# medical-genomics-group/ci-gwas

Measured on AMD Instinct MI355X. Metric: ci_tests_per_sec, higher is better.
Workload: dtype f32; 1 GPU; cusk level sweep, one LD block 10000 SNPs x 20 traits, N=16384, alpha=0.0001, max level 5 (north_star headline); correlation matrix from synthetic .bed (Kendall-npn/Pearson) resident in HBM; n_variables=10020, engine=cusk

## Files before the change

### ci-gwas_amd/csrc/cusk_internal.h

```cpp
#pragma once
#include <hip/hip_runtime.h>

#include <cstdint>
#include <cstdio>
#include <string>
#include <vector>

#include "../../include/cusk_hip.h"

namespace cusk {

constexpr int kML = CUSK_ML;
constexpr int kLevels = CUSK_ML + 2;
constexpr unsigned long long kNone = ~0ull;
constexpr int kNumClasses = 5;
constexpr int kClassCap[kNumClasses] = {39, 63, 127, 191, 1 << 30};
constexpr int kThreads = 256;
constexpr int kTmajMinLevelDefault = 6;
constexpr int kCounterSlots = 512;
constexpr size_t kLdsLimit = 160 * 1024;

struct DevBuf
{
    void *p = nullptr;
    size_t cap = 0;
    hipError_t ensure(size_t bytes)
    {
        if (bytes <= cap) return hipSuccess;
        if (p) (void)hipFree(p);
        p = nullptr;
        cap = 0;
        size_t want = bytes + bytes / 4 + 256;
        hipError_t e = hipMalloc(&p, want);
        if (e == hipSuccess) cap = want;
        return e;
    }
    void release()
    {
        if (p) (void)hipFree(p);
        p = nullptr;
        cap = 0;
    }
    template <typename T>
    T *as() const
    {
        return reinterpret_cast<T *>(p);
    }
};

struct LevelCounters;
struct HostGate;

}

struct cusk_engine
{
    int device = 0;
    hipStream_t stream = nullptr;
    hipStream_t stream2 = nullptr;
    hipStream_t stream3 = nullptr;
    float *mxp_pinned = nullptr;
    size_t mxp_pinned_cap = 0, mxp_pending = 0;
    hipEvent_t ev_fork = nullptr, ev_join = nullptr, ev_z = nullptr;
    hipEvent_t ev_mxp = nullptr;
    bool own_stream = false;
    std::string err;

    int n = 0;
    int words = 0;
    int mode = -1;
    bool have_result = false;
    cusk::DevBuf adj, adj0;
    cusk::DevBuf deg, binom, counters, slots, rec_base, ti, queue, symflag;
    cusk::DevBuf off[2], nbr[2], best[2];
    cusk::DevBuf planblk;
    unsigned plan_seq = 0;
    cusk::DevBuf off1;
    cusk::DevBuf items[2][cusk::kNumClasses];
    cusk::DevBuf rec_x, rec_y, rec_l, rec_s;
    long long rec_cap = 0;
    long long rec_slots = 0;
    cusk::DevBuf den_x, den_y, den_l, den_z, den_s, den_counts, den_off;
    long long den_stride = 0;
    bool records_ready = false, z_ready = false;
    cusk::DevBuf scratch_a, scratch_b;
    const float *last_C = nullptr;
    int last_levels = 0;
    std::vector<int> batch_lo, batch_hi;
    cusk::DevBuf row_range, row_blk, blk_woff;
    void *batch_pinned = nullptr;
    size_t batch_pinned_cap = 0;
    void *res_pinned = nullptr;
    size_t res_pinned_cap = 0;
    cusk::DevBuf rv, rpos, sel, wpre;
    cusk::DevBuf nv;
    int level1_form = -1;
    long long nrec = 0;
    cusk::LevelCounters *hcnt = nullptr;
    unsigned long long *hslots = nullptr;
    long long *hrec_base = nullptr;
    unsigned long long *hcanon = nullptr;
    int *hflag = nullptr;
    std::vector<unsigned long long> binom_host;
    long long binom_rows = 0;
    cusk::HostGate *hgate = nullptr, *hgate_dev = nullptr;
    int run_seq = 0;
    long long item_cap_cur = 0;
    hipEvent_t ev_main[2] = {nullptr, nullptr};
    hipEvent_t ev_run[2] = {nullptr, nullptr};
    hipEvent_t ev_k0[cusk::kLevels], ev_k1[cusk::kLevels], ev_l0[cusk::kLevels], ev_l1[cusk::kLevels];

    int opt_fast = 1;
    int opt_validate = 0;
    int opt_het_filter = 0;
    int opt_het_rows = 0;
    int opt_corr_fp4 = 1;
    int opt_pair = 1;
    int opt_rows = 1;
    int opt_vec = 1;
    int opt_overlap = 1;
    int opt_corr_popcount = 0;
    int opt_corr_mxp_f32 = 0;
    int opt_assume_symmetric = 0;
    long long opt_queue_cap = 4ll << 20;
    int opt_hostprof = 0;
    int opt_tmaj_validate_stride = 1;
    int opt_max_staged_classes = -1;
    int opt_tmaj_min_level = cusk::kTmajMinLevelDefault;
    long long opt_chunk = 2048;
    long long opt_chunk0 = 512;
    long long opt_chunk0_low = 256;
    int opt_vec_threads = 64;
    long long opt_item_cap = 1ll << 20;
    int opt_lookahead = 2;
    int opt_sync2 = 1;
    int opt_l1_threads = 0;
    int opt_l1_lds_row = 1;
    int opt_timing = 1;
    long long opt_sep_ws_budget = 4ll << 30;

    int shard_rank = 0, shard_world = 1;
    int shard_host_staging = 0;
    cusk_exchange_fn shard_fn = nullptr;
    void *shard_user = nullptr;
    void *shard_host = nullptr;
    size_t shard_host_cap = 0;

    cusk::DevBuf bed_dev, phen_dev, mean_dev, std_dev, planes, mxp_dev, pxp_dev, mxp_bq;
    cusk::DevBuf pc_masks, pc_counts;
    cusk::DevBuf mp_bits;
    cusk::DevBuf corr_tab[2];
    void *corr_tab_pinned[2] = {nullptr, nullptr};
    size_t corr_tab_pinned_cap[2] = {0, 0};
    hipEvent_t ev_corr[5] = {nullptr, nullptr, nullptr, nullptr, nullptr};
    float corr_ms[4] = {0, 0, 0, 0};
};

namespace cusk {

inline int fail(cusk_engine *e, int code, const std::string &msg)
{
    if (e) e->err = msg;
    return code;
}

#define CUSK_HIP(e, call)                                                                        \
    do                                                                                           \
    {                                                                                            \
        hipError_t _st = (call);                                                                 \
        if (_st != hipSuccess)                                                                   \
            return cusk::fail((e), CUSK_ERR_HIP,                                                 \
                              std::string(#call) + ": " + hipGetErrorString(_st) + " (" +        \
                                  __FILE__ + ":" + std::to_string(__LINE__) + ")");              \
    } while (0)

void threshold_array_host(int n, float alpha, float *thr15);
float hetcor_threshold_host(float alpha);

int corr_build_impl(cusk_engine *e, const unsigned char *bed, const float *phen, size_t m, size_t N,
                    size_t p, const float *mean, const float *std, float *C_dev, float *mxp_host,
                    float *mxm_tri_host, float *pxp_tri_host, bool ahead = false);
bool is_device_pointer(const void *p);

int check_marker_ix(cusk_engine *e, const int *marker_ix, size_t k, size_t m_total);
int pack_bed_rows(cusk_engine *e, const unsigned char *bed, const int *marker_ix, const int *&ix_d, size_t k, size_t m_total,
                  size_t clb, std::vector<unsigned char> &bed_h, const unsigned char *&bed_k);

void compat_marker_phen_corr_pearson(const unsigned char *marker_vals, const float *phen_vals, const size_t num_markers,
                                     const size_t num_individuals, const size_t num_phen, const float *marker_mean,
                                     const float *marker_std, float *marker_phen_corrs);
void compat_corr_pearson_npn(const unsigned char *marker_vals, const float *phen_vals, const size_t num_markers,
                             const size_t num_individuals, const size_t num_phen, const float *marker_mean,
                             const float *marker_std, float *marker_corrs, float *marker_phen_corrs, float *phen_corrs);
double qnorm_host(double p);

}
```

### ci-gwas_amd/csrc/engine.hip

```cpp
#include <algorithm>
#include <atomic>
#include <chrono>
#include <cmath>
#include <cstdlib>
#include <cstring>

#include "sweep_common.h"

namespace cusk {

static unsigned long long binom_sat(int n, int k)
{
    if (k < 0 || k > n) return 0;
    if (k > n - k) k = n - k;
    unsigned long long r = 1;
    const unsigned long long cap = 1ull << 62;
    for (int i = 1; i <= k; i++)
    {
        unsigned long long f = (unsigned long long)(n - k + i);
        if (r > cap / f) return cap;
        r = r * f / (unsigned long long)i;
    }
    return r;
}
// ... 253 lines not shown
        CUSK_HIP(e, launch_finalize(l, pl.fp, s));
        return CUSK_OK;
    };

    auto shard_join = [&](int l) -> int {
        LevelPlan &pl = plan[l];
        if (pl.use_fast && l >= 2)
        {
            CUSK_HIP(e, hipMemcpyAsync(e->hcnt + l, dcnt + l, sizeof(LevelCounters), hipMemcpyDeviceToHost, s));
            CUSK_HIP(e, hipStreamSynchronize(s));
            if (e->hcnt[l].qcount > (unsigned long long)e->opt_queue_cap)
            {
                pl.redone = true;
                local.exact_fallbacks++;
                qcap_gate[l] = ~0ull;
                const int rc = launch_level_sweeps(l, true);
                if (rc != CUSK_OK) return rc;
            }
        }
        const size_t count = (size_t)e->hgate[l].total_edges;
        if (a.mode == 1 && !pl.use_rows) CUSK_HIP(e, launch_marks_from_bitmap(pl.sp, e->sel.as<unsigned>(), s));
        const int elem = (pl.use_rows || a.mode == 1) ? 4 : 8;
        void *dev = (pl.use_rows || a.mode == 1) ? e->sel.p : e->best[l & 1].p;
        int rc = 0;
        if (e->shard_host_staging)
        {
            const size_t bytes = count * (size_t)elem;
            if (bytes > e->shard_host_cap)
            {
                if (e->shard_host) (void)hipHostFree(e->shard_host);
                e->shard_host = nullptr;
                e->shard_host_cap = 0;
                CUSK_HIP(e, hipHostMalloc(&e->shard_host, std::max<size_t>(bytes, 64)));
                e->shard_host_cap = std::max<size_t>(bytes, 64);
            }
            CUSK_HIP(e, hipMemcpyAsync(e->shard_host, dev, bytes, hipMemcpyDeviceToHost, s));
            CUSK_HIP(e, hipStreamSynchronize(s));
            rc = e->shard_fn(e->shard_user, l, e->shard_host, count, elem, 0, (void *)s);
            if (rc == 0) CUSK_HIP(e, hipMemcpyAsync(dev, e->shard_host, bytes, hipMemcpyHostToDevice, s));
        }
        else
        {
            CUSK_HIP(e, hipStreamSynchronize(s));
            rc = e->shard_fn(e->shard_user, l, dev, count, elem, 1, (void *)s);
        }
        if (rc != 0) return fail(e, CUSK_ERR_ARG, "row-shard exchange failed at level " + std::to_string(l));
        if (a.mode == 1)
            CUSK_HIP(e, launch_level1_apply(pl.sp, e->sel.as<unsigned>(), (l == 1 && pl.use_rows) ? e->rpos.p : nullptr, false, s));
        return CUSK_OK;
    };

    if (last_level >= 1 && !a.row_range)
        CUSK_HIP(e, launch_degree(e->adj.as<unsigned long long>(), e->deg.as<int>(), n, words,
                                  a.mode == 0 ? e->adj0.as<unsigned long long>() : nullptr, s));

    int staged_classes = 0;
    while (staged_classes < kNumClasses - 1 && lds_layout(kClassCap[staged_classes], het).total <= kLdsLimit) staged_classes++;
    if (e->opt_max_staged_classes >= 0) staged_classes = std::min(staged_classes, e->opt_max_staged_classes);
    const int lookahead = sharded ? 0 : std::max(0, e->opt_lookahead);
    auto wait_gate = [&](int l) -> int {
        volatile int *seq = &e->hgate[l].seq;
        for (unsigned long it = 1; *seq != run_seq; it++)
        {
            if ((it & 0x3fff) == 0)
            {
                const hipError_t q = hipStreamQuery(s);
                if (q == hipSuccess)
                {
                    if (*seq == run_seq) break;
                    return fail(e, CUSK_ERR_HIP, "level " + std::to_string(l) + ": the stream drained without the level's gate record");
                }
                if (q != hipErrorNotReady) return fail(e, CUSK_ERR_HIP, std::string("stream error while waiting for a level gate: ") + hipGetErrorString(q));
            }
            __builtin_ia32_pause();
        }
        std::atomic_thread_fence(std::memory_order_acquire);
        return CUSK_OK;
    };
    int maxdeg1 = 0;
    int maxdeg2 = -1;
    int start = 1;
    int redo = 0;
    bool first_pass = true;

    for (;;)
    {
        if (redo > 0)
        {
            plan[redo].redone = true;
            local.exact_fallbacks++;
            qcap_gate[redo] = ~0ull;
            int rc = launch_level_sweeps(redo, true);
            if (rc != CUSK_OK) return rc;
            rc = launch_level_finalize(redo);
            if (rc != CUSK_OK) return rc;
            if (e->opt_timing == 2) CUSK_HIP(e, hipEventRecord(e->ev_l1[redo], s));
            redo = 0;
        }
        int enq_last = start - 1;
        int planned_last = start - 1;
        for (int l = start; l <= last_level; l++)
        {
            const int cs = l & 1;
            {
                const int k = l - 1 - lookahead;
                if (k >= start)
                {
                    const int rc = wait_gate(k);
                    if (rc != CUSK_OK) return rc;
                    if (!e->hgate[k].active) break;
                }
            }
            if (e->opt_timing == 2) CUSK_HIP(e, hipEventRecord(e->ev_l0[l], s));
            LevelPlan &pl = plan[l];
            pl.redone = false;
            pl.known_items = false;
            const bool first_build = (l == 1 && first_pass);
            int *off_l = (l == 1) ? e->off1.as<int>() : e->off[cs].as<int>();
            PlanArgs pa;
            pa.deg = e->deg.as<int>();
            pa.off = off_l;
            for (int c = 0; c < kNumClasses; c++) pa.items[c] = e->items[cs][c].as<int2>();
            pa.n = n;
            pa.L = l;
            pa.binom = e->binom.as<unsigned long long>();
            pa.chunk = chunk;
            {
                float th_l;
                if (het)
                    th_l = a.Th[0];
                else if (a.mode == 0)
                    th_l = a.Th[l];
                else
                    th_l = uniform_ess_threshold(a.Th[0], a.ess_uniform, l);
                const bool vec0 = (e->opt_fast != 0) && l >= 2 && l < kVecMaxLevel && th_l >= kThMinFilter && !het && e->opt_vec &&
                                  !e->opt_validate && staged_classes > 0;
                const unsigned long long c0 = (l <= 4) ? (unsigned long long)std::max<long long>(e->opt_chunk0_low, 64) : chunk0;
                plan[l].chunk0 = vec0 ? c0 : chunk;
                plan[l].tmaj = (e->opt_fast != 0) && !plan[l].force_exact && l >= std::max(2, e->opt_tmaj_min_level) && l <= kML &&
                               th_l >= kThMinFilter && (!het || ness_symmetric) && symmetric && !sharded;
                if (plan[l].tmaj) plan[l].chunk0 = chunk;
            }
            pa.chunk0 = plan[l].chunk0;
            pa.Lsets = plan[l].tmaj ? l + 1 : l;
            pa.staged_classes = staged_classes;
            pa.pair_mode = ((l == 1) && !first_build && plan[l].use_pair && !plan[l].use_rows) ? 1 : 0;
            pa.cnt = dcnt + l;
            pa.prev = (l >= 2) ? dcnt + (l - 1) : nullptr;
            pa.prev_qcap = (l >= 2) ? qcap_gate[l - 1] : ~0ull;
            pa.item_cap = item_cap;
            pa.shard_rank = e->shard_rank;
            pa.shard_world = e->shard_world;
            pa.gate = e->hgate_dev + l;
            pa.seq = run_seq;
            pa.sym = (l == 1 && !e->opt_assume_symmetric && !a.row_range) ? dsym : nullptr;
            pa.blocks = e->planblk.as<unsigned long long>();
            pa.blk_seq = ++e->plan_seq;
            if (first_build && e->binom_rows <= 0)
            {
                CUSK_HIP(e, e->binom.ensure(sizeof(unsigned long long) * kBinomStride));
                pa.binom = e->binom.as<unsigned long long>();
            }
            CUSK_HIP(e, launch_plan(pa, s));
            planned_last = l;
            if (first_build)
            {
                hp_mark("plan1_enq");
                int *const rec_l_before = (a.mode == 0) ? e->rec_l.as<int>() : nullptr;
                const size_t rec_l_cleared = rec_l_before ? e->rec_l.cap : 0;
                if (rec_l_cleared) CUSK_HIP(e, hipMemsetAsync(rec_l_before, 0, rec_l_cleared, s));
                int rc = wait_gate(1);
                if (rc != CUSK_OK) return rc;
                hp_mark("gate1");
                symmetric = (e->hgate[1].sym == 0) || (e->opt_assume_symmetric != 0) || (a.row_range != nullptr);
                ness_symmetric = ness_checked && (*reinterpret_cast<volatile int *>(e->hflag) == 0);
                ness_symmetric_rows = ness_checked_rows && (*reinterpret_cast<volatile int *>(e->hflag) == 0);
                cap_edges = std::max<long long>(e->hgate[1].total_edges, 1);
                maxdeg1 = e->hgate[1].maxdeg;
                for (int k = 0; k < 2; k++)
                {
                    CUSK_HIP(e, e->nbr[k].ensure(sizeof(int) * ((size_t)cap_edges + 4)));
                    if (a.mode == 0) CUSK_HIP(e, e->best[k].ensure(sizeof(unsigned long long) * (size_t)cap_edges));
                }
                CUSK_HIP(e, e->rv.ensure(sizeof(float) * ((size_t)cap_edges + 4)));
                CUSK_HIP(e, e->rpos.ensure(sizeof(int) * 4 * (size_t)cap_edges));
                CUSK_HIP(e, e->sel.ensure(sizeof(unsigned) * (size_t)cap_edges));
                if (a.mode == 0)
                {
                    CUSK_HIP(e, e->rec_x.ensure(sizeof(int) * (size_t)cap_edges));
                    CUSK_HIP(e, e->rec_y.ensure(sizeof(int) * (size_t)cap_edges));
                    CUSK_HIP(e, e->rec_l.ensure(sizeof(int) * (size_t)cap_edges));
                    CUSK_HIP(e, e->rec_s.ensure(sizeof(int) * kML * (size_t)cap_edges));
                    e->rec_cap = (long long)(e->rec_l.cap / sizeof(int));
                    if ((long long)(e->rec_s.cap / (sizeof(int) * kML)) < e->rec_cap) e->rec_cap = (long long)(e->rec_s.cap / (sizeof(int) * kML));
                    e->rec_slots = cap_edges;
                    if (e->rec_l.as<int>() != rec_l_before || rec_l_cleared < sizeof(int) * (size_t)cap_edges)
                        CUSK_HIP(e, hipMemsetAsync(e->rec_l.p, 0, sizeof(int) * (size_t)cap_edges, s));
                    CUSK_HIP(e, e->wpre.ensure(sizeof(int) * (size_t)n * words));
                }
                CUSK_HIP(e, e->queue.ensure(sizeof(RecheckEntry) * (size_t)e->opt_queue_cap));
                if ((long long)maxdeg1 >= e->binom_rows)
                {
                    const int rows = std::max(maxdeg1 + 1, 1024);
                    e->binom_host.assign((size_t)rows * kBinomStride, 0ull);
                    for (int aa = 0; aa < rows; aa++)
                        for (int b = 0; b < kBinomStride; b++)
                            e->binom_host[(size_t)aa * kBinomStride + b] = binom_sat(aa, b);
                    CUSK_HIP(e, e->binom.ensure(e->binom_host.size() * sizeof(unsigned long long)));
                    CUSK_HIP(e, hipMemcpyAsync(e->binom.p, e->binom_host.data(),
                                               e->binom_host.size() * sizeof(unsigned long long), hipMemcpyHostToDevice, s));
                    e->binom_rows = rows;
                }
                pl.pair_lds = (size_t)maxdeg1 * 20 + 16;
                pl.use_pair = !het && symmetric && (e->opt_pair != 0) && pl.pair_lds <= 64 * 1024;
                pl.use_rows = !het && symmetric && (e->opt_pair != 0) && (e->opt_rows != 0);
                if (het0 && ness_symmetric_rows && symmetric && (e->opt_fast != 0) && (e->opt_pair != 0) && (e->opt_rows != 0))
                {
                    pl.use_rows = true;
                    CUSK_HIP(e, e->nv.ensure(sizeof(float) * ((size_t)cap_edges + 4)));
                }
                if (pl.use_rows) CUSK_HIP(e, e->wpre.ensure(sizeof(int) * (size_t)n * words));
                if (pl.use_pair && !pl.use_rows)
                {
                    CUSK_HIP(e, hipMemsetAsync(dcnt + l, 0, sizeof(LevelCounters), s));
                    pa.pair_mode = 1;
                    pa.binom = e->binom.as<unsigned long long>();
                    pa.seq = run_seq;
                    e->hgate[1].seq = 0;
                    pa.blk_seq = ++e->plan_seq;
                    CUSK_HIP(e, launch_plan(pa, s));
                }
                first_pass = false;
            }
            if (sharded)
            {
                const int rc = wait_gate(l);
                if (rc != CUSK_OK) return rc;
                if (!e->hgate[l].active) break;
                for (int c = 0; c < kNumClasses; c++) pl.nitems[c] = e->hgate[l].class_items[c];
                pl.known_items = true;
            }
            pl.use_fast = (e->opt_fast != 0) && (l >= 2) && !pl.force_exact && !het0_exact;
            CUSK_HIP(e, launch_fill_nbr(e->adj.as<unsigned long long>(), off_l, e->nbr[cs].as<int>(),
                                        (a.mode == 0 && !pl.use_rows) ? e->best[cs].as<unsigned long long>() : nullptr, n, words,
                                        (l == 1 && (pl.use_rows || a.mode == 0)) ? e->wpre.as<int>() : nullptr, dcnt + l, a.row_range, s));
            if (l == 2 && !sharded && e->opt_sync2)
            {
                const int rc2 = wait_gate(2);
                if (rc2 != CUSK_OK) return rc2;
                if (!e->hgate[2].active) break;
                for (int c = 0; c < kNumClasses; c++) pl.nitems[c] = e->hgate[2].class_items[c];
                pl.known_items = !e->hgate[2].item_overflow;
                maxdeg2 = e->hgate[2].maxdeg;
            }
            {
                pl.maxdeg_bound = maxdeg1;
                if (maxdeg2 >= 0 && l >= 2) pl.maxdeg_bound = std::min(pl.maxdeg_bound, maxdeg2);
                const int k = l - 1 - lookahead;
                if (k >= 1 && e->hgate[k].seq == run_seq && e->hgate[k].active) pl.maxdeg_bound = std::min(pl.maxdeg_bound, e->hgate[k].maxdeg);
                pl.staged_classes = staged_classes;
            }

            SweepParams &sp = pl.sp;
            sp.C = a.C;
            sp.Ness = a.Ness;
            sp.n = n;
            sp.level = l;
            sp.off = off_l;
            sp.nbr = e->nbr[cs].as<int>();
            sp.best = e->best[cs].as<unsigned long long>();
            sp.adj = e->adj.as<unsigned long long>();
            sp.deg = e->deg.as<int>();
            sp.words = words;
            sp.items = nullptr;
            sp.binom = e->binom.as<unsigned long long>();
            sp.time_index = e->ti.as<int>();
            sp.has_ti = (a.mode == 1 && a.time_index != nullptr) ? 1 : 0;
            sp.chunk = chunk;
            sp.cap = 0;
            sp.cls = 0;
            sp.item_cap = item_cap;
            sp.grid_cap = item_cap;
            sp.cnt = dcnt + l;
            sp.row_range = a.row_range;
            sp.max_span = a.row_range ? a.max_span : n;
            sp.slots = dslots + (size_t)l * kCounterSlots * 4;
            if (het)
                sp.th = a.Th[0];
            else if (a.mode == 0)
                sp.th = a.Th[l];
            else
                sp.th = uniform_ess_threshold(a.Th[0], a.ess_uniform, l);
            {
                const double tq = std::tanh((double)sp.th);
                sp.t2 = (float)(tq * tq);
                pl.filter_ok = (sp.th >= kThMinFilter);
                if (!pl.filter_ok) pl.use_fast = false;
            }
            sp.queue = nullptr;
            sp.qcap = 0;
            qcap_gate[l] = ~0ull;
            if (pl.use_fast)
            {
                sp.queue = e->queue.as<RecheckEntry>();
                sp.qcap = (unsigned long long)e->opt_queue_cap;
                qcap_gate[l] = sp.qcap;
            }
            FinalizeParams &fp = pl.fp;
            fp.C = a.C;
            fp.n = n;
            fp.off = sp.off;
            fp.nbr = sp.nbr;
            fp.best = sp.best;
            fp.sel = pl.use_rows ? e->sel.as<unsigned>() : nullptr;
            fp.level = l;
            fp.adj = sp.adj;
            fp.deg = sp.deg;
            fp.words = words;
            fp.binom = sp.binom;
            fp.off1 = e->off1.as<int>();
            fp.wpre1 = e->wpre.as<int>();
            fp.adj0 = e->adj0.as<unsigned long long>();
            fp.rec_x = e->rec_x.as<int>();
            fp.rec_y = e->rec_y.as<int>();
            fp.rec_l = e->rec_l.as<int>();
            fp.rec_s = e->rec_s.as<int>();
            fp.rec_cap = e->rec_cap;
            fp.meta = pl.use_rows ? e->rpos.as<int4>() : nullptr;
            fp.cnt = dcnt + l;
            fp.qcap = qcap_gate[l];
            fp.slots = sp.slots;
            fp.canon = dcanon + (size_t)l * kCounterSlots;

            if (e->opt_timing == 1 || e->opt_timing == 2) CUSK_HIP(e, hipEventRecord(e->ev_k0[l], s));
            int rc = launch_level_sweeps(l, false);
            if (rc != CUSK_OK) return rc;
            if (e->opt_timing == 1 || e->opt_timing == 2) CUSK_HIP(e, hipEventRecord(e->ev_k1[l], s));
            if (sharded)
            {
                rc = shard_join(l);
                if (rc != CUSK_OK) return rc;
            }
            rc = launch_level_finalize(l);
            if (rc != CUSK_OK) return rc;
            if (e->opt_timing == 2) CUSK_HIP(e, hipEventRecord(e->ev_l1[l], s));
            enq_last = l;
        }

        CUSK_HIP(e, hipEventRecord(e->ev_join, e->stream2));
        CUSK_HIP(e, hipStreamWaitEvent(s, e->ev_join, 0));
        CUSK_HIP(e, hipMemcpyAsync(e->hcnt, ctl, ctl_sym, hipMemcpyDeviceToHost, s));
        CUSK_HIP(e, hipEventRecord(e->ev_run[1], s));
        hp_mark("all_enq");
        CUSK_HIP(e, hipStreamSynchronize(s));
        hp_mark("synced");
        int ended = 0;
        for (int l = 1; l <= planned_last && !ended; l++)
            if (!e->hcnt[l].active) ended = l;
        const int last_ran = ended ? ended - 1 : enq_last;
        if (!sharded && last_ran >= 2 && plan[last_ran].use_fast && !plan[last_ran].redone &&
            e->hcnt[last_ran].qcount > (unsigned long long)e->opt_queue_cap)
        {
            if (plan[last_ran].tmaj)
            {
                plan[last_ran].force_exact = true;
                local.exact_fallbacks++;
                start = last_ran;
            }
            else
            {
                redo = last_ran;
                start = last_ran + 1;
            }
        }
        else if (ended && e->hcnt[ended].overflow)
            return fail(e, CUSK_ERR_OVERFLOW,
                        "C(degree, level) exceeds 2^62 at level " + std::to_string(ended) + " (max degree " +
                            std::to_string(e->hcnt[ended].maxdeg) + ")");
        else if (ended && e->hcnt[ended].item_overflow)
        {
            long long need = item_cap;
            for (int c = 0; c < kNumClasses; c++) need = std::max(need, e->hcnt[ended].class_items[c]);
            item_cap = need + need / 4;
            for (int k = 0; k < 2; k++)
                for (int c = 0; c < kNumClasses; c++) CUSK_HIP(e, e->items[k][c].ensure(sizeof(int2) * (size_t)item_cap));
            start = ended;
        }
        else
        {
            levels_swept = last_ran;
            if (ended) level_out = ended - 1;
            break;
        }
        for (int l = start; l < kLevels; l++) e->hgate[l].seq = 0;
        if (start <= 2) maxdeg2 = -1;
        if (start <= last_level)
        {
            CUSK_HIP(e, hipMemsetAsync(dcnt + start, 0, sizeof(LevelCounters) * (size_t)(kLevels - start), s));
            CUSK_HIP(e, hipMemsetAsync(dslots + (size_t)start * kCounterSlots * 4, 0,
                                       sizeof(unsigned long long) * (size_t)(kLevels - start) * kCounterSlots * 4, s));
            CUSK_HIP(e, hipMemsetAsync(dcanon + (size_t)start * kCounterSlots, 0,
                                       sizeof(unsigned long long) * (size_t)(kLevels - start) * kCounterSlots, s));
        }
    }
    for (int l = 1; l <= std::min(levels_swept + 1, last_level); l++)
    {
        local.max_degree[l] = e->hcnt[l].maxdeg;
        local.edges[l] = e->hcnt[l].total_edges;
    }
    local.levels_run += levels_swept;
    float ms = 0.0f;
    CUSK_HIP(e, hipEventElapsedTime(&ms, e->ev_l0[0], e->ev_l1[0]));
    local.kernel_ms[0] = local.level_ms[0] = ms;
    const bool timed = (e->opt_timing == 1 || e->opt_timing == 2);
    for (int l = 1; l <= levels_swept; l++)
    {
        for (int k = 0; k < kCounterSlots; k++)
        {
            const unsigned long long *sl = e->hslots + ((size_t)l * kCounterSlots + k) * 4;
            local.tests[l] += (long long)sl[0];
            local.subsets[l] += (long long)sl[1];
            local.removed[l] += (long long)sl[2];
            local.violations += (long long)sl[3];
            if (a.mode == 0 || l == 1) local.canonical_tests[l] += (long long)e->hcanon[(size_t)l * kCounterSlots + k];
        }
        local.rechecks[l] = (long long)e->hcnt[l].qcount;
        if (!timed)
        {
            if (e->opt_timing == 3 && l == 1 && rows_timed)
            {
                CUSK_HIP(e, hipEventElapsedTime(&ms, e->ev_main[0], e->ev_main[1]));
                local.main_kernel_ms[l] = ms;
            }
            continue;
        }
        CUSK_HIP(e, hipEventElapsedTime(&ms, e->ev_k0[l], e->ev_k1[l]));
        local.kernel_ms[l] = ms;
        local.main_kernel_ms[l] = ms;
        if (l == 1 && rows_timed)
        {
            CUSK_HIP(e, hipEventElapsedTime(&ms, e->ev_main[0], e->ev_main[1]));
            local.main_kernel_ms[l] = ms;
        }
// ... 127 lines not shown
    if (e->shard_host) (void)hipHostFree(e->shard_host);
    if (e->hcnt) (void)hipHostFree(e->hcnt);
    if (e->hflag) (void)hipHostFree(e->hflag);
    if (e->hgate) (void)hipHostFree(e->hgate);
    for (auto &ev : e->ev_run)
        if (ev) (void)hipEventDestroy(ev);
    for (auto &ev : e->ev_main)
        if (ev) (void)hipEventDestroy(ev);
    for (auto &ev : e->ev_corr)
        if (ev) (void)hipEventDestroy(ev);
    for (int l = 0; l < kLevels; l++)
        for (hipEvent_t ev : {e->ev_k0[l], e->ev_k1[l], e->ev_l0[l], e->ev_l1[l]})
            if (ev) (void)hipEventDestroy(ev);
    for (hipEvent_t ev : {e->ev_fork, e->ev_join, e->ev_z, e->ev_mxp})
        if (ev) (void)hipEventDestroy(ev);
    if (e->stream2) (void)hipStreamDestroy(e->stream2);
    if (e->stream3) (void)hipStreamDestroy(e->stream3);
    if (e->mxp_pinned) (void)hipHostFree(e->mxp_pinned);
    if (e->own_stream && e->stream) (void)hipStreamDestroy(e->stream);
    delete e;
}

extern "C" int cusk_engine_set_option(cusk_engine *e, const char *key, long long value)
{
    if (!e || !key) return CUSK_ERR_ARG;
    const std::string k(key);
    if (k == "fast")
        e->opt_fast = (int)value;
    else if (k == "validate")
        e->opt_validate = (int)value;
    else if (k == "het_filter")
        e->opt_het_filter = (int)value;
    else if (k == "het_rows" && (value == 0 || value == 1))
        e->opt_het_rows = (int)value;
    else if (k == "corr_fp4")
        e->opt_corr_fp4 = (int)value;
    else if (k == "pair")
        e->opt_pair = (int)value;
    else if (k == "rows")
        e->opt_rows = (int)value;
    else if (k == "vec")
        e->opt_vec = (int)value;
    else if (k == "overlap")
        e->opt_overlap = (int)value;
    else if (k == "corr_popcount")
        e->opt_corr_popcount = (int)value;
    else if (k == "corr_mxp_f32")
        e->opt_corr_mxp_f32 = (int)value;
    else if (k == "assume_symmetric")
        e->opt_assume_symmetric = (int)value;
    else if (k == "queue_capacity" && value > 0)
        e->opt_queue_cap = value;
    else if (k == "chunk" && value >= 256)
        e->opt_chunk = value;
    else if (k == "max_staged_classes")
        e->opt_max_staged_classes = (int)value;
    else if (k == "tmaj_validate_stride" && value >= 1 && (value & (value - 1)) == 0)
        e->opt_tmaj_validate_stride = (int)value;
    else if (k == "tmaj_min_level")
        e->opt_tmaj_min_level = (int)value;
    else if (k == "hostprof")
        e->opt_hostprof = (int)value;
    else if (k == "chunk0_low" && value >= 64)
        e->opt_chunk0_low = value;
    else if (k == "chunk0" && value >= 64)
        e->opt_chunk0 = value;
    else if (k == "vec_threads" && (value == 64 || value == 128 || value == 256))
        e->opt_vec_threads = (int)value;
    else if (k == "item_capacity" && value > 0)
    {
        e->opt_item_cap = value;
        e->item_cap_cur = 0;
    }
    else if (k == "lookahead" && value >= 0)
        e->opt_lookahead = (int)value;
    else if (k == "timing")
        e->opt_timing = (int)value;
    else if (k == "l1_threads" && (value == 0 || value == 256 || value == 512))
        e->opt_l1_threads = (int)value;
    else if (k == "l1_lds_row" && (value == 0 || value == 1))
        e->opt_l1_lds_row = (int)value;
    else if (k == "sync2")
        e->opt_sync2 = (int)value;
    else if (k == "sepselect_ws_bytes" && value > 0)
        e->opt_sep_ws_budget = value;
    else
        return fail(e, CUSK_ERR_ARG, "unknown option " + k);
    return CUSK_OK;
}

extern "C" int cusk_engine_set_row_shard(cusk_engine *e, int rank, int world, cusk_exchange_fn fn, void *user, int host_staging)
{
    if (!e) return CUSK_ERR_ARG;
    if (world < 1 || rank < 0 || rank >= world || (world > 1 && !fn))
        return fail(e, CUSK_ERR_ARG, "cusk_engine_set_row_shard: need 0 <= rank < world and an exchange function");
    e->shard_rank = rank;
    e->shard_world = world;
    e->shard_fn = fn;
    e->shard_user = user;
    e->shard_host_staging = host_staging ? 1 : 0;
    return CUSK_OK;
}

extern "C" const char *cusk_last_error(const cusk_engine *e) { return e ? e->err.c_str() : "no engine"; }
extern "C" void *cusk_engine_stream(const cusk_engine *e) { return e ? (void *)e->stream : nullptr; }
extern "C" int cusk_engine_device(const cusk_engine *e) { return e ? e->device : -1; }
extern "C" int cusk_engine_level1_form(const cusk_engine *e) { return e ? e->level1_form : -1; }
extern "C" int cusk_engine_bind_thread(cusk_engine *e)
{
    if (!e) return CUSK_ERR_ARG;
    CUSK_HIP(e, hipSetDevice(e->device));
    return CUSK_OK;
}

extern "C" int cusk_run_skeleton(cusk_engine *e, const float *C_dev, int n, const float *Th, int maxlevel,
                                 cusk_stats *stats)
{
    if (!e) return CUSK_ERR_ARG;
    e->batch_lo.clear();
    RunArgs a{};
    a.mode = 0;
    a.C = C_dev;
    a.Th = Th;
    a.n = n;
    a.maxlevel = maxlevel;
    return run_levels(e, a, stats);
}

static int batch_setup(cusk_engine *e, const char *who, int n, int nblk, const int *lo, const int *hi, RunArgs &a)
{
    int prev = 0, span = 0;
    long long pairs0 = 0;
    for (int b = 0; b < nblk; b++)
    {
        if ((lo[b] & 63) != 0 || lo[b] < prev || hi[b] < lo[b] || hi[b] > n)
            return fail(e, CUSK_ERR_ARG, std::string(who) + ": block bases must be ascending multiples of 64 inside the matrix");
        prev = hi[b];
        span = std::max(span, hi[b] - lo[b]);
        pairs0 += (long long)(hi[b] - lo[b]) * (hi[b] - lo[b] - 1) / 2;
    }
    CUSK_HIP(e, hipSetDevice(e->device));
    const size_t bytes_rr = sizeof(int2) * (size_t)n, bytes_rb = sizeof(int) * (size_t)n, bytes_wo = sizeof(long long) * (size_t)nblk;
    const size_t need = bytes_rr + bytes_rb + bytes_wo;
    if (need > e->batch_pinned_cap)
    {
        if (e->batch_pinned) (void)hipHostFree(e->batch_pinned);
        e->batch_pinned = nullptr;
        e->batch_pinned_cap = 0;
        CUSK_HIP(e, hipHostMalloc(&e->batch_pinned, need + need / 2));
        e->batch_pinned_cap = need + need / 2;
    }
    int2 *rr = static_cast<int2 *>(e->batch_pinned);
    int *rb = reinterpret_cast<int *>(static_cast<char *>(e->batch_pinned) + bytes_rr);
    long long *wo = reinterpret_cast<long long *>(static_cast<char *>(e->batch_pinned) + bytes_rr + bytes_rb);
    for (int r = 0; r < n; r++)
    {
        rr[r] = make_int2(0, 0);
        rb[r] = -1;
    }
    long long woff = 0;
    for (int b = 0; b < nblk; b++)
    {
        for (int r = lo[b]; r < hi[b]; r++)
        {
            rr[r] = make_int2(lo[b], hi[b]);
            rb[r] = b;
        }
        wo[b] = woff;
        woff += (long long)(hi[b] - lo[b]) * ((hi[b] - lo[b] + 63) / 64);
    }
    CUSK_HIP(e, e->row_range.ensure(bytes_rr));
    CUSK_HIP(e, e->row_blk.ensure(bytes_rb));
    CUSK_HIP(e, e->blk_woff.ensure(bytes_wo));
    CUSK_HIP(e, hipMemcpyAsync(e->row_range.p, rr, bytes_rr, hipMemcpyHostToDevice, e->stream));
    CUSK_HIP(e, hipMemcpyAsync(e->row_blk.p, rb, bytes_rb, hipMemcpyHostToDevice, e->stream));
    CUSK_HIP(e, hipMemcpyAsync(e->blk_woff.p, wo, bytes_wo, hipMemcpyHostToDevice, e->stream));
    e->batch_lo.assign(lo, lo + nblk);
    e->batch_hi.assign(hi, hi + nblk);
    a.row_range = e->row_range.as<int2>();
    a.max_span = span;
    a.level0_pairs = pairs0;
    return CUSK_OK;
}

extern "C" int cusk_run_skeleton_batch(cusk_engine *e, const float *C_dev, int n, int nblk, const int *lo, const int *hi,
                                       const float *Th, int maxlevel, cusk_stats *stats)
{
    if (!e) return CUSK_ERR_ARG;
    if (!C_dev || !lo || !hi || !Th || n <= 0 || nblk <= 0) return fail(e, CUSK_ERR_ARG, "bad arguments");
    if (e->shard_world > 1) return fail(e, CUSK_ERR_ARG, "batched runs are not row-sharded");
// ... 418 lines not shown
```

### ci-gwas_amd/csrc/plan.hip

```cpp
#include "sweep_common.h"

namespace cusk {


__global__ void degree_kernel(const unsigned long long *__restrict__ adj, int *deg, int n, int words, unsigned long long *adj0)
{
    const int row = blockIdx.x * (blockDim.x >> 6) + (threadIdx.x >> 6);
    const int lane = threadIdx.x & 63;
    if (row >= n) return;
    int d = 0;
    for (int w = lane; w < words; w += 64)
    {
        const unsigned long long v = adj[(size_t)row * words + w];
        if (adj0) adj0[(size_t)row * words + w] = v;
        d += __popcll(v);
    }
    for (int o = 32; o > 0; o >>= 1) d += __shfl_xor(d, o);
    if (lane == 0) deg[row] = d;
}

hipError_t launch_degree(const unsigned long long *adj, int *deg, int n, int words, unsigned long long *adj0, hipStream_t st)
{
    hipLaunchKernelGGL(degree_kernel, dim3((n + 3) / 4), dim3(256), 0, st, adj, deg, n, words, adj0);
    return hipGetLastError();
// ... 23 lines not shown
        int incl = c;
        for (int o = 1; o < 64; o <<= 1)
        {
            const int v = __shfl_up(incl, o);
            if (lane >= o) incl += v;
        }
        int pos = o0 + run + incl - c;
        if (wpre && w < w_end) wpre[(size_t)row * words + w] = run + incl - c;
        while (bits)
        {
            const int b = __ffsll((long long)bits) - 1;
            bits &= bits - 1;
            if (best) best[pos] = kNone;
            nbr[pos++] = w * 64 + b;
        }
        run += __shfl(incl, 63);
    }
}

hipError_t launch_fill_nbr(const unsigned long long *adj, const int *off, int *nbr, unsigned long long *best, int n, int words,
                           int *wpre, const LevelCounters *cnt, const int2 *row_range, hipStream_t st)
{
    hipLaunchKernelGGL(fill_nbr_kernel, dim3((n + 3) / 4), dim3(256), 0, st, adj, off, nbr, best, n, words, wpre, cnt, row_range);
    return hipGetLastError();
}

__device__ __forceinline__ long long prefix_256(const int *__restrict__ in, int n, int v, long long *s_red, long long *block_total)
{
    const int tid = threadIdx.x, lane = tid & 63, wave = tid >> 6;
    const int first = blockIdx.x * 256;
    long long before = 0;
    for (int i0 = 0; i0 < first; i0 += 256 * 16)
    {
        int t[16];
#pragma unroll
        for (int u = 0; u < 16; u++)
        {
            const int i = i0 + u * 256 + tid;
            t[u] = (i < first) ? in[i] : 0;
        }
#pragma unroll
        for (int u = 0; u < 16; u++) before += t[u];
    }
    int incl = v;
    for (int o = 1; o < 64; o <<= 1)
    {
        const int t = __shfl_up(incl, o);
        if (lane >= o) incl += t;
    }
    for (int o = 32; o > 0; o >>= 1) before += __shfl_xor(before, o);
    if (lane == 63) s_red[wave] = incl;
    if (lane == 0) s_red[4 + wave] = before;
    __syncthreads();
    long long pre = s_red[4] + s_red[5] + s_red[6] + s_red[7];
    for (int w = 0; w < wave; w++) pre += s_red[w];
    *block_total = s_red[0] + s_red[1] + s_red[2] + s_red[3];
    (void)n;
    return pre + incl - v;
}

constexpr int kPlanWords = 8;
static_assert(kNumClasses + 1 < 7, "plan words");
constexpr unsigned long long kPlanMask = (1ull << 40) - 1ull;

__global__ void __launch_bounds__(256) plan_kernel(PlanArgs a)
{
    __shared__ long long s_wave[kNumClasses][4];
    __shared__ int s_wdeg[4], s_wmax[4];
    __shared__ long long s_part[4][kPlanWords];
    __shared__ long long s_base[kNumClasses];
    __shared__ int s_cls[256], s_nch[256], s_pos[256];
    __shared__ unsigned long long s_big[4];
    LevelCounters *cnt = a.cnt;
    const int n = a.n, L = a.L;
    if (a.prev != nullptr && !level_complete(a.prev, a.prev_qcap))
    {
        if (blockIdx.x == 0 && threadIdx.x == 0)
        {
            HostGate *g = a.gate;
            g->active = 0;
            g->maxdeg = 0;
            g->overflow = 0;
            g->item_overflow = 0;
            g->sym = 0;
            g->total_edges = 0;
            for (int c = 0; c < kNumClasses; c++) g->class_items[c] = 0;
            __threadfence_system();
            *(volatile int *)&g->seq = a.seq;
        }
        return;
    }
    const int tid = threadIdx.x;
    const int row = blockIdx.x * 256 + tid;
    const int lane = tid & 63, wave = tid >> 6;
    int cls = -1, nchunks = 0;
    const int d = (row < n) ? a.deg[row] : 0;
    bool ovf = false;
    if (d > L)
    {
        const unsigned long long nc = a.pair_mode ? (unsigned long long)d * (d - 1) / 2
                                                  : (L == 1 ? (unsigned long long)d : a.binom[(size_t)d * kBinomStride + a.Lsets]);
        if (nc >= (1ull << 62))
            ovf = true;
        else
        {
            cls = 0;
            while (d > kClassCap[cls]) cls++;
            if (cls >= a.staged_classes) cls = kNumClasses - 1;
            const unsigned long long ch = (cls == 0) ? a.chunk0 : a.chunk;
            if (a.Lsets == L + 1 && L >= 2)
            {
                const int np = L - 2;
                long long tot = 0;
                for (int s = np; s <= d - 3; s++)
                {
                    const unsigned long long nP = (np == 0) ? 1ull : a.binom[(size_t)s * kBinomStride + np];
                    const unsigned long long per = (unsigned long long)kThreads * tmaj_prefixes_per_lane(d, s, ch);
                    tot += (long long)((nP + per - 1ull) / per);
                }
                if (tot > (long long)0x7fffffff)
                    ovf = true;
                else
                    nchunks = (int)tot;
            }
            else
            {
                const unsigned long long units = (nc + ch - 1) / ch;
                if (units > 0x7fffffffull)
                    ovf = true;
                else
                    nchunks = (int)units;
            }
            if (ovf || !(a.shard_world == 1 || row % a.shard_world == a.shard_rank))
            {
                cls = -1;
                nchunks = 0;
            }
        }
    }
    const bool wave_ovf = __ballot(ovf) != 0ull;
    int dincl = d, dmax = d;
    for (int o = 1; o < 64; o <<= 1)
    {
        const int t = __shfl_up(dincl, o);
        if (lane >= o) dincl += t;
    }
    for (int o = 32; o > 0; o >>= 1) dmax = max(dmax, __shfl_xor(dmax, o));
    if (lane == 63) s_wdeg[wave] = dincl;
    if (lane == 0) s_wmax[wave] = dmax | (wave_ovf ? (1 << 30) : 0);
    long long excl[kNumClasses];
#pragma unroll
    for (int c = 0; c < kNumClasses; c++)
    {
        const long long mine = (cls == c) ? nchunks : 0;
        long long v = mine;
        for (int o = 1; o < 64; o <<= 1)
        {
            const long long t = __shfl_up(v, o);
            if (lane >= o) v += t;
        }
        excl[c] = v - mine;
        if (lane == 63) s_wave[c][wave] = v;
    }
    __syncthreads();
    unsigned long long *blk = a.blocks + (size_t)blockIdx.x * kPlanWords;
    const unsigned long long tag = (unsigned long long)a.blk_seq << 40;
// ... 24 lines not shown
        }
        for (int o = 8; o < 64; o <<= 1)
        {
            const long long t = __shfl_xor(acc, o);
            acc = (w >= 6) ? max(acc, t) : acc + t;
        }
        if (lane < kPlanWords) s_part[wave][lane] = acc;
    }
    __syncthreads();
    long long before[kPlanWords];
#pragma unroll
    for (int w = 0; w < kPlanWords; w++)
    {
        const long long p0 = s_part[0][w], p1 = s_part[1][w], p2 = s_part[2][w], p3 = s_part[3][w];
        before[w] = (w >= 6) ? max(max(p0, p1), max(p2, p3)) : p0 + p1 + p2 + p3;
    }
    {
        long long o0 = before[0] + dincl - d;
        for (int w = 0; w < wave; w++) o0 += s_wdeg[w];
        if (row < n) a.off[row] = (int)o0;
    }
    const bool last = (blockIdx.x == gridDim.x - 1);
    long long tot_items[kNumClasses];
#pragma unroll
    for (int c = 0; c < kNumClasses; c++)
    {
        const long long mine = s_wave[c][0] + s_wave[c][1] + s_wave[c][2] + s_wave[c][3];
        tot_items[c] = before[1 + c] + mine;
        if (tid == c) s_base[c] = (tot_items[c] > a.item_cap) ? -1 : before[1 + c];
    }
    __syncthreads();
    {
        int pos = -1;
        if (cls >= 0 && s_base[cls] >= 0)
        {
            long long add = 0;
            for (int w = 0; w < wave; w++) add += s_wave[cls][w];
            long long e = 0;
#pragma unroll
            for (int c = 0; c < kNumClasses; c++)
                if (cls == c) e = excl[c];
            pos = (int)(s_base[cls] + add + e);
        }
        const bool big = (pos >= 0 && nchunks > 1);
        if (pos >= 0 && nchunks == 1) a.items[cls][pos] = make_int2(row, 0);
        const unsigned long long bm = __ballot(big);
        if (lane == 0) s_big[wave] = bm;
        if (big)
        {
            s_cls[tid] = cls;
            s_nch[tid] = nchunks;
            s_pos[tid] = pos;
        }
        __syncthreads();
        const int row0 = blockIdx.x * 256;
        for (int w = 0; w < 4; w++)
        {
            unsigned long long m = s_big[w];
            while (m)
            {
                const int r = w * 64 + __builtin_ctzll(m);
                m &= m - 1;
                const int nch = s_nch[r];
                int2 *dst = a.items[s_cls[r]] + s_pos[r];
                for (int c = tid; c < nch; c += 256) dst[c] = make_int2(row0 + r, c);
            }
        }
    }
    if (last && tid == 0)
    {
        const long long edges = before[0] + s_wdeg[0] + s_wdeg[1] + s_wdeg[2] + s_wdeg[3];
        const int maxdeg = (int)max(before[6], (long long)(max(max(s_wmax[0], s_wmax[1]), max(s_wmax[2], s_wmax[3])) & ~(1 << 30)));
        a.off[n] = (int)edges;
        const int ovf_all = (before[7] != 0 || (((s_wmax[0] | s_wmax[1] | s_wmax[2] | s_wmax[3]) >> 30) & 1)) ? 1 : 0;
        cnt->overflow = ovf_all;
        bool fits = true;
        HostGate *g = a.gate;
        for (int c = 0; c < kNumClasses; c++)
        {
            fits = fits && (tot_items[c] <= a.item_cap);
            cnt->class_items[c] = tot_items[c];
            g->class_items[c] = tot_items[c];
        }
        const int active = (maxdeg - 1 >= L && ovf_all == 0 && fits) ? 1 : 0;
        cnt->maxdeg = maxdeg;
        cnt->total_edges = edges;
        cnt->item_overflow = fits ? 0 : 1;
        cnt->active = active;
        g->active = active;
        g->maxdeg = maxdeg;
        g->overflow = ovf_all;
        g->item_overflow = fits ? 0 : 1;
        g->sym = a.sym ? *a.sym : 0;
        g->total_edges = edges;
        __threadfence_system();
        *(volatile int *)&g->seq = a.seq;
    }
}

hipError_t launch_plan(const PlanArgs &a, hipStream_t st)
{
    hipLaunchKernelGGL(plan_kernel, dim3((a.n + 255) / 256), dim3(256), 0, st, a);
    return hipGetLastError();
}

}
```

### ci-gwas_amd/csrc/sweep_common.h

```cpp
#pragma once
#include "cusk_internal.h"

namespace cusk {

constexpr int kBinomStride = 16;
constexpr int kVecMaxLevel = 9;
constexpr float kThMinFilter = 2e-3f;

struct RowInfo
{
    int cls;
    int base;
    int nchunks;
    int pad;
};

struct RecheckEntry
{
    int x;
    int k2;
    unsigned long long rank;
};

struct LevelCounters
{
    int maxdeg;
    int overflow;
    long long total_edges;
    long long class_items[kNumClasses];
    unsigned long long qcount;
    unsigned long long rec_total;
    int active;
    int item_overflow;
    unsigned int done_blocks;
    int pad;
    unsigned long long next_item[kNumClasses];
};

struct HostGate
{
    int seq;
    int active, maxdeg, overflow, item_overflow, sym;
    long long total_edges;
    long long class_items[kNumClasses];
};

struct SweepParams
{
    const float *C;
    const float *Ness;
    int n;
    int level;
    const int *off;
    const int *nbr;
    unsigned long long *best;
    unsigned long long *adj;
    int *deg;
    int words;
    const int2 *items;
    const unsigned long long *binom;
    const int *time_index;
    int has_ti;
    float th;
    float t2;
    unsigned long long chunk;
    int cap;
    int cls;
    long long item_cap;
    long long grid_cap;
    LevelCounters *cnt;
    unsigned long long *slots;
    RecheckEntry *queue;
    unsigned long long qcap;
    int validate;
    const int2 *row_range;
    int max_span;
};

struct FinalizeParams
{
    const float *C;
    int n;
    const int *off;
    const int *nbr;
    const unsigned long long *best;
    const unsigned *sel;
    int level;
    unsigned long long *adj;
    int *deg;
    int words;
    const unsigned long long *binom;
    const int *off1;
    const int *wpre1;
    const unsigned long long *adj0;
    int *rec_x, *rec_y, *rec_l, *rec_s;
    long long rec_cap;
    const int4 *meta;
    const LevelCounters *cnt;
    unsigned long long qcap;
    unsigned long long *slots;
    unsigned long long *canon;
};

__host__ __device__ inline size_t align16(size_t x) { return (x + 15) & ~(size_t)15; }

struct LdsLayout
{
    size_t nbr, best, ti, sub, ess, total;
};
__host__ __device__ inline LdsLayout lds_layout(int cap, bool het)
{
    LdsLayout l;
    size_t ld = (size_t)((cap + 1) | 1);
    l.nbr = 0;
    l.best = align16(l.nbr + sizeof(int) * (cap + 1));
    l.ti = align16(l.best + sizeof(unsigned long long) * cap);
    l.sub = align16(l.ti + sizeof(int) * (cap + 1));
    l.ess = align16(l.sub + sizeof(float) * (cap + 1) * ld);
    l.total = het ? align16(l.ess + sizeof(float) * (cap + 1) * ld) : l.ess;
    return l;
}

#if defined(__HIPCC__)
__device__ __forceinline__ long long level_items(const SweepParams &p)
{
// ... 46 lines not shown
#pragma unroll
    for (int i = 0; i < L; i++)
    {
        const int lo = prev + 1, hi = S[i] - 1;
        const int t = L - i - 1;
        if (lo <= hi)
        {
            if (in_prefix)
                cnt += C(d - lo, t + 1) - C(d - 1 - hi, t + 1);
            else if (k > prev)
            {
                const int h2 = min(hi, k - 1);
                if (t >= 1 && lo <= h2) cnt += C(d - 1 - lo, t) - C(d - 2 - h2, t);
                if (lo <= k && k <= hi) cnt += C(d - 1 - k, t);
            }
        }
        if (S[i] == k) in_prefix = true;
        prev = S[i];
    }
    return cnt + (in_prefix ? 1ull : 0ull);
}

__device__ __forceinline__ bool clear_edge(unsigned long long *adj, int *deg, int words, int X, int Y)
{
    const unsigned long long o1 = atomicAnd(&adj[(size_t)X * words + (Y >> 6)], ~(1ull << (Y & 63)));
    const unsigned long long o2 = atomicAnd(&adj[(size_t)Y * words + (X >> 6)], ~(1ull << (X & 63)));
    const bool f1 = (o1 >> (Y & 63)) & 1ull, f2 = (o2 >> (X & 63)) & 1ull;
    if (f1) atomicSub(&deg[X], 1);
    if (f2) atomicSub(&deg[Y], 1);
    return f1;
}
#endif

hipError_t launch_sweep_exact(int mode, bool het, int L, const SweepParams &p, int cls, hipStream_t st);
hipError_t launch_recheck(int mode, bool het, int L, const SweepParams &p, hipStream_t st);
hipError_t launch_finalize(int L, const FinalizeParams &p, hipStream_t st);
hipError_t launch_record_z(int L, const float *C, int n, const int *x, const int *y, const int *l, const int *s, long long stride,
                           long long count, float *z, hipStream_t st);
constexpr int kRecBlock = 1024;
hipError_t launch_rec_count(const int *rec_l, long long slots, int *counts, hipStream_t st);
hipError_t launch_rec_compact(const int *rec_l, const int *rec_x, const int *rec_y, const int *rec_s, long long rec_cap,
                              long long slots, const long long *block_off, int *out_x, int *out_y, int *out_l, int *out_s,
                              long long out_stride, hipStream_t st);
hipError_t launch_sweep_fast(int mode, bool het, int L, bool validate, const SweepParams &p, int cls, hipStream_t st);
hipError_t launch_sweep_tmaj(int mode, bool het, int L, const SweepParams &p, int cls, hipStream_t st);
hipError_t launch_ess_symmetry(const float *N, int n, const int2 *row_range, int *flag, hipStream_t st);
__host__ __device__ inline int tmaj_prefixes_per_lane(int d, int s, unsigned long long chunk)
{
    const unsigned long long r = (unsigned long long)(d - 1 - s);
    const unsigned long long pairs = r * (r - 1ull) / 2ull;
    const unsigned long long k = chunk / ((unsigned long long)kThreads * (pairs ? pairs : 1ull));
    return (int)(k < 1ull ? 1ull : (k > 64ull ? 64ull : k));
}
hipError_t launch_sweep_vec(int mode, int L, const SweepParams &p, int cls, int threads, hipStream_t st);
unsigned persistent_grid(const void *kernel, int threads, size_t lds);
size_t sweep_vec_lds_bytes(int cls);
hipError_t launch_level0(const float *C, const float *Ness, const int *Ginit, unsigned long long *adj, int n, int words,
                         float th, int *asym_flag, hipStream_t st);
hipError_t launch_level0_batch(const float *C, const float *Ness, unsigned long long *adj, unsigned long long *adj0, int *deg, int n,
                               int words, const int2 *row_range, float th, hipStream_t st);
hipError_t launch_degree(const unsigned long long *adj, int *deg, int n, int words, unsigned long long *adj0, hipStream_t st);
hipError_t launch_fill_nbr(const unsigned long long *adj, const int *off, int *nbr, unsigned long long *best, int n, int words,
                           int *wpre, const LevelCounters *cnt, const int2 *row_range, hipStream_t st);
struct PlanArgs
{
    const int *deg;
    int *off;
    int2 *items[kNumClasses];
    int n, L;
    int Lsets;
    const unsigned long long *binom;
    unsigned long long chunk, chunk0;
    int staged_classes, pair_mode;
    LevelCounters *cnt;
    const LevelCounters *prev;
    unsigned long long prev_qcap;
    long long item_cap;
    int shard_rank, shard_world;
    HostGate *gate;
    int seq;
    const int *sym;
    unsigned long long *blocks;
    unsigned blk_seq;
};
hipError_t launch_plan(const PlanArgs &a, hipStream_t st);
hipError_t launch_expand_records(const int *rec_s, const int *rec_l, long long rec_cap, long long count, int *out,
                                 hipStream_t st);
hipError_t launch_level1_rows(int mode, bool validate, bool use_filter, const SweepParams &p, float *rv, void *meta,
                              unsigned *sel, const int *wpre, hipEvent_t ev_begin, hipEvent_t ev_end, int shard_rank,
                              int shard_world, int force_threads, bool lds_row, bool defer_apply, bool has_ti,
                              unsigned long long *canon, hipStream_t st, float *nv = nullptr, int *form = nullptr);
hipError_t launch_marks_from_bitmap(const SweepParams &p, unsigned *sel, hipStream_t st);
hipError_t launch_level1_apply(const SweepParams &p, const unsigned *sel, const void *meta, bool count_removed, hipStream_t st);
hipError_t launch_pair(int mode, const SweepParams &p, size_t lds, hipStream_t st);
hipError_t launch_gather_sub(const float *M, int n, const int *idx, int k, float *out, hipStream_t st);
hipError_t launch_gather_rows(const float *M, int n, const int *idx, const int *row_src, const int *row_k, const long long *row_first,
                              const long long *row_out, long long nrows, float *out, hipStream_t st);
hipError_t launch_pack_block_bits(const unsigned long long *adj, int n, int words, const int2 *row_range, const int *row_blk,
                                  const long long *blk_woff, unsigned long long *out, int tail, hipStream_t st);
hipError_t launch_expand_adj(const unsigned long long *adj, int *G, int n, int words, hipStream_t st);
hipError_t launch_expand_pmax(const unsigned long long *adj, const unsigned long long *adj0, const float *C, float *pmax,
                              int n, int words, const int *x, const int *y, const float *z, long long nrec, hipStream_t st);

}
```

Measured before the change: 253.0 billion CI tests/s.

## Speculatively skip level-1 host gate wait using prior buffer capacities

```diff
diff --git a/ci-gwas_amd/csrc/cusk_internal.h b/ci-gwas_amd/csrc/cusk_internal.h
--- a/ci-gwas_amd/csrc/cusk_internal.h
+++ b/ci-gwas_amd/csrc/cusk_internal.h
@@ -103,6 +103,8 @@
     int *hflag = nullptr;
     std::vector<unsigned long long> binom_host;
     long long binom_rows = 0;
+    int maxdeg1_last = 0;
+    int level1_setup = -1;
     cusk::HostGate *hgate = nullptr, *hgate_dev = nullptr;
     int run_seq = 0;
     long long item_cap_cur = 0;
@@ -136,6 +138,8 @@
     int opt_sync2 = 1;
     int opt_l1_threads = 0;
     int opt_l1_lds_row = 1;
+    int opt_l1_spec = 1;
+    int opt_binom_floor = 1024;
     int opt_timing = 1;
     long long opt_sep_ws_budget = 4ll << 30;
 
@@ -156,6 +160,8 @@
     float corr_ms[4] = {0, 0, 0, 0};
 };
 
+extern "C" int cusk_engine_level1_setup(const cusk_engine *e);
+
 namespace cusk {
 
 inline int fail(cusk_engine *e, int code, const std::string &msg)
diff --git a/ci-gwas_amd/csrc/engine.hip b/ci-gwas_amd/csrc/engine.hip
--- a/ci-gwas_amd/csrc/engine.hip
+++ b/ci-gwas_amd/csrc/engine.hip
@@ -359,6 +359,44 @@
     int start = 1;
     int redo = 0;
     bool first_pass = true;
+    e->level1_setup = -1;
+    bool spec_allowed = e->opt_l1_spec != 0 && !sharded && !het && (e->opt_assume_symmetric != 0 || a.row_range != nullptr) &&
+                        e->opt_pair != 0 && e->opt_rows != 0 && e->binom_rows > 0;
+    bool spec_pending = false;
+    bool spec_overflow = false;
+    auto spec_capacity = [&]() -> long long {
+        long long cap = (long long)(e->rv.cap / sizeof(float)) - 4;
+        for (int k = 0; k < 2; k++)
+        {
+            cap = std::min(cap, (long long)(e->nbr[k].cap / sizeof(int)) - 4);
+            if (a.mode == 0) cap = std::min(cap, (long long)(e->best[k].cap / sizeof(unsigned long long)));
+        }
+        cap = std::min(cap, (long long)(e->rpos.cap / (sizeof(int) * 4)));
+        cap = std::min(cap, (long long)(e->sel.cap / sizeof(unsigned)));
+        if (a.mode == 0)
+        {
+            for (const DevBuf *b : {&e->rec_x, &e->rec_y, &e->rec_l}) cap = std::min(cap, (long long)(b->cap / sizeof(int)));
+            cap = std::min(cap, (long long)(e->rec_s.cap / (sizeof(int) * kML)));
+        }
+        if (e->wpre.cap < sizeof(int) * (size_t)n * words) cap = 0;
+        if (e->queue.cap < sizeof(RecheckEntry) * (size_t)e->opt_queue_cap) cap = 0;
+        return std::max<long long>(cap, 0);
+    };
+    auto resolve_spec = [&]() -> int {
+        const int rc = wait_gate(1);
+        if (rc != CUSK_OK) return rc;
+        hp_mark("gate1");
+        spec_pending = false;
+        if (e->hgate[1].cap_overflow)
+        {
+            spec_overflow = true;
+            return CUSK_OK;
+        }
+        cap_edges = std::max<long long>(e->hgate[1].total_edges, 1);
+        maxdeg1 = e->maxdeg1_last = e->hgate[1].maxdeg;
+        if (a.mode == 0) e->rec_slots = cap_edges;
+        return CUSK_OK;
+    };
 
     for (;;)
     {
@@ -383,9 +421,10 @@
                 const int k = l - 1 - lookahead;
                 if (k >= start)
                 {
-                    const int rc = wait_gate(k);
+                    int rc = wait_gate(k);
                     if (rc != CUSK_OK) return rc;
-                    if (!e->hgate[k].active) break;
+                    if (spec_pending && (rc = resolve_spec()) != CUSK_OK) return rc;
+                    if (spec_overflow || !e->hgate[k].active) break;
                 }
             }
             if (e->opt_timing == 2) CUSK_HIP(e, hipEventRecord(e->ev_l0[l], s));
@@ -433,16 +472,41 @@
             pa.sym = (l == 1 && !e->opt_assume_symmetric && !a.row_range) ? dsym : nullptr;
             pa.blocks = e->planblk.as<unsigned long long>();
             pa.blk_seq = ++e->plan_seq;
+            pa.edge_cap = -1;
+            pa.binom_rows = e->binom_rows;
             if (first_build && e->binom_rows <= 0)
             {
                 CUSK_HIP(e, e->binom.ensure(sizeof(unsigned long long) * kBinomStride));
                 pa.binom = e->binom.as<unsigned long long>();
             }
+            const long long spec_cap = (first_build && spec_allowed) ? spec_capacity() : 0;
+            if (spec_cap > 0) pa.edge_cap = spec_cap;
             CUSK_HIP(e, launch_plan(pa, s));
             planned_last = l;
-            if (first_build)
+            if (first_build && spec_cap > 0)
             {
                 hp_mark("plan1_enq");
+                if (a.mode == 0) CUSK_HIP(e, hipMemsetAsync(e->rec_l.p, 0, e->rec_l.cap, s));
+                symmetric = true;
+                cap_edges = spec_cap;
+                maxdeg1 = e->maxdeg1_last;
+                if (a.mode == 0)
+                {
+                    e->rec_cap = (long long)(e->rec_l.cap / sizeof(int));
+                    if ((long long)(e->rec_s.cap / (sizeof(int) * kML)) < e->rec_cap) e->rec_cap = (long long)(e->rec_s.cap / (sizeof(int) * kML));
+                    e->rec_slots = spec_cap;
+                }
+                pl.pair_lds = (size_t)maxdeg1 * 20 + 16;
+                pl.use_pair = pl.pair_lds <= 64 * 1024;
+                pl.use_rows = true;
+                spec_pending = true;
+                e->level1_setup = 1;
+                first_pass = false;
+            }
+            else if (first_build)
+            {
+                hp_mark("plan1_enq");
+                if (e->level1_setup < 0) e->level1_setup = 0;
                 int *const rec_l_before = (a.mode == 0) ? e->rec_l.as<int>() : nullptr;
                 const size_t rec_l_cleared = rec_l_before ? e->rec_l.cap : 0;
                 if (rec_l_cleared) CUSK_HIP(e, hipMemsetAsync(rec_l_before, 0, rec_l_cleared, s));
@@ -453,7 +517,7 @@
                 ness_symmetric = ness_checked && (*reinterpret_cast<volatile int *>(e->hflag) == 0);
                 ness_symmetric_rows = ness_checked_rows && (*reinterpret_cast<volatile int *>(e->hflag) == 0);
                 cap_edges = std::max<long long>(e->hgate[1].total_edges, 1);
-                maxdeg1 = e->hgate[1].maxdeg;
+                maxdeg1 = e->maxdeg1_last = e->hgate[1].maxdeg;
                 for (int k = 0; k < 2; k++)
                 {
                     CUSK_HIP(e, e->nbr[k].ensure(sizeof(int) * ((size_t)cap_edges + 4)));
@@ -478,7 +542,7 @@
                 CUSK_HIP(e, e->queue.ensure(sizeof(RecheckEntry) * (size_t)e->opt_queue_cap));
                 if ((long long)maxdeg1 >= e->binom_rows)
                 {
-                    const int rows = std::max(maxdeg1 + 1, 1024);
+                    const int rows = std::max(maxdeg1 + 1, std::max(e->opt_binom_floor, 1));
                     e->binom_host.assign((size_t)rows * kBinomStride, 0ull);
                     for (int aa = 0; aa < rows; aa++)
                         for (int b = 0; b < kBinomStride; b++)
@@ -521,6 +585,12 @@
             CUSK_HIP(e, launch_fill_nbr(e->adj.as<unsigned long long>(), off_l, e->nbr[cs].as<int>(),
                                         (a.mode == 0 && !pl.use_rows) ? e->best[cs].as<unsigned long long>() : nullptr, n, words,
                                         (l == 1 && (pl.use_rows || a.mode == 0)) ? e->wpre.as<int>() : nullptr, dcnt + l, a.row_range, s));
+            if (l == 2 && spec_pending)
+            {
+                const int rcs = resolve_spec();
+                if (rcs != CUSK_OK) return rcs;
+                if (spec_overflow) break;
+            }
             if (l == 2 && !sharded && e->opt_sync2)
             {
                 const int rc2 = wait_gate(2);
@@ -631,11 +701,24 @@
         hp_mark("all_enq");
         CUSK_HIP(e, hipStreamSynchronize(s));
         hp_mark("synced");
+        if (spec_pending)
+        {
+            const int rcs = resolve_spec();
+            if (rcs != CUSK_OK) return rcs;
+        }
         int ended = 0;
         for (int l = 1; l <= planned_last && !ended; l++)
             if (!e->hcnt[l].active) ended = l;
         const int last_ran = ended ? ended - 1 : enq_last;
-        if (!sharded && last_ran >= 2 && plan[last_ran].use_fast && !plan[last_ran].redone &&
+        if (spec_overflow)
+        {
+            spec_overflow = false;
+            spec_allowed = false;
+            first_pass = true;
+            e->level1_setup = 2;
+            start = 1;
+        }
+        else if (!sharded && last_ran >= 2 && plan[last_ran].use_fast && !plan[last_ran].redone &&
             e->hcnt[last_ran].qcount > (unsigned long long)e->opt_queue_cap)
         {
             if (plan[last_ran].tmaj)
@@ -929,6 +1012,10 @@
         e->opt_l1_lds_row = (int)value;
     else if (k == "sync2")
         e->opt_sync2 = (int)value;
+    else if (k == "l1_spec" && (value == 0 || value == 1))
+        e->opt_l1_spec = (int)value;
+    else if (k == "binom_floor" && value >= 1 && value <= (1 << 20))
+        e->opt_binom_floor = (int)value;
     else if (k == "sepselect_ws_bytes" && value > 0)
         e->opt_sep_ws_budget = value;
     else
@@ -953,6 +1040,7 @@
 extern "C" void *cusk_engine_stream(const cusk_engine *e) { return e ? (void *)e->stream : nullptr; }
 extern "C" int cusk_engine_device(const cusk_engine *e) { return e ? e->device : -1; }
 extern "C" int cusk_engine_level1_form(const cusk_engine *e) { return e ? e->level1_form : -1; }
+extern "C" int cusk_engine_level1_setup(const cusk_engine *e) { return e ? e->level1_setup : -1; }
 extern "C" int cusk_engine_bind_thread(cusk_engine *e)
 {
     if (!e) return CUSK_ERR_ARG;
diff --git a/ci-gwas_amd/csrc/plan.hip b/ci-gwas_amd/csrc/plan.hip
--- a/ci-gwas_amd/csrc/plan.hip
+++ b/ci-gwas_amd/csrc/plan.hip
@@ -129,6 +129,7 @@
             g->maxdeg = 0;
             g->overflow = 0;
             g->item_overflow = 0;
+            g->cap_overflow = 0;
             g->sym = 0;
             g->total_edges = 0;
             for (int c = 0; c < kNumClasses; c++) g->class_items[c] = 0;
@@ -319,7 +320,8 @@
             cnt->class_items[c] = tot_items[c];
             g->class_items[c] = tot_items[c];
         }
-        const int active = (maxdeg - 1 >= L && ovf_all == 0 && fits) ? 1 : 0;
+        const int cap_ovf = (a.edge_cap >= 0 && (edges > a.edge_cap || (long long)maxdeg >= a.binom_rows)) ? 1 : 0;
+        const int active = (maxdeg - 1 >= L && ovf_all == 0 && fits && cap_ovf == 0) ? 1 : 0;
         cnt->maxdeg = maxdeg;
         cnt->total_edges = edges;
         cnt->item_overflow = fits ? 0 : 1;
@@ -328,6 +330,7 @@
         g->maxdeg = maxdeg;
         g->overflow = ovf_all;
         g->item_overflow = fits ? 0 : 1;
+        g->cap_overflow = cap_ovf;
         g->sym = a.sym ? *a.sym : 0;
         g->total_edges = edges;
         __threadfence_system();
diff --git a/ci-gwas_amd/csrc/sweep_common.h b/ci-gwas_amd/csrc/sweep_common.h
--- a/ci-gwas_amd/csrc/sweep_common.h
+++ b/ci-gwas_amd/csrc/sweep_common.h
@@ -41,6 +41,8 @@
 {
     int seq;
     int active, maxdeg, overflow, item_overflow, sym;
+    int cap_overflow;
+    int pad;
     long long total_edges;
     long long class_items[kNumClasses];
 };
@@ -253,6 +255,8 @@
     const int *sym;
     unsigned long long *blocks;
     unsigned blk_seq;
+    long long edge_cap;
+    long long binom_rows;
 };
 hipError_t launch_plan(const PlanArgs &a, hipStream_t st);
 hipError_t launch_expand_records(const int *rec_s, const int *rec_l, long long rec_cap, long long count, int *out,
```

New measurement: 252.6 billion CI tests/s. No clear change (-0.1%).
